# TXH-mercury/VALOR

Hardware: AMD Instinct MI355X
Metric: pretrain samples/sec (V+A+T clip) (higher is better)
Workload: dtype bf16

## Files before the change

include/valor_hip.h:

```cpp
#ifndef VALOR_HIP_H
#define VALOR_HIP_H
#include <stdint.h>
#ifdef __cplusplus
extern "C" {
#endif

#define VALOR_DT_BF16 0
#define VALOR_DT_F32 1
#define VALOR_OK 0
#define VALOR_ERR_ARG (-1)
#define VALOR_ERR_LAUNCH (-2)
#define VALOR_ACT_NONE 0
#define VALOR_ACT_GELU_ERF 1
#define VALOR_ACT_QUICK_GELU 2
#define VALOR_ACT_RELU 3
#define VALOR_ACT_TANH 4
#define VALOR_ACT_DERIV 16

int valor_gemm(void* stream, int dtype, int transA, int transB, int M, int N, int K, const void* A, int64_t lda,
               const void* B, int64_t ldb, void* C, int64_t ldc, const void* bias, int act, void* preact,
               const void* dact_aux, int64_t ldaux, float alpha, int accumulate, int out_f32, void* workspace,
               int64_t workspace_bytes, void* rowsum_out,
               int rowsum_accumulate);

typedef struct valor_gemm_policy {
    int key[12];
    int variant;
    int tr_asm;
    int fast_epilogue;
    int sched_256;
    int sched_narrow;
} valor_gemm_policy;
int valor_gemm_tuned(const valor_gemm_policy* policy, void* stream, int dtype, int transA, int transB, int M, int N, int K,
                     const void* A, int64_t lda, const void* B, int64_t ldb, void* C, int64_t ldc, const void* bias, int act,
                     void* preact, const void* dact_aux, int64_t ldaux, float alpha, int accumulate, int out_f32, void* workspace,
                     int64_t workspace_bytes, void* rowsum_out, int rowsum_accumulate);
int valor_gemm_kernel_for_tuned(const valor_gemm_policy* policy, int dtype, int transA, int transB, int M, int N, int K,
                                int heavy_epilogue);

typedef struct valor_gemm_pending { unsigned char opaque[256]; } valor_gemm_pending;
int valor_gemm_deferred(void* stream, int dtype, int transA, int transB, int M, int N, int K, const void* A, int64_t lda,
                        const void* B, int64_t ldb, void* C, int64_t ldc, const void* bias, int act, void* preact,
                        const void* dact_aux, int64_t ldaux, float alpha, int accumulate, int out_f32, void* workspace,
                        int64_t workspace_bytes, void* rowsum_out, int rowsum_accumulate, valor_gemm_pending* pending);
int valor_gemm_pending_bytes(const valor_gemm_pending* pending, int64_t* bytes);
int valor_gemm_reduce_group(void* stream, int dtype, const valor_gemm_pending* pendings, int n);

int valor_gemm_set_variant(int v);
int valor_gemm_kernel_for(int dtype, int transA, int transB, int M, int N, int K, int heavy_epilogue);
int valor_gemm_set_tr_asm(int v);
int valor_gemm_set_fast_epilogue(int v);
int valor_gemm_set_policy(int key, int value);
int valor_gemm_set_8ph_sched(int v);
int valor_gemm_set_narrow_sched(int v);
int valor_gemm_narrow_occupancy(void);
int valor_gemm_wide_occupancy(void);

typedef struct valor_xattn_seg {
    const void* q; const void* o; const void* dout; void* dq; const float* lse; const int* kv_range;
    int64_t q_bs, q_rs, o_bs, o_rs, do_bs, do_rs, dq_bs, dq_rs;
    int B, Sq;
    uint64_t seed, offset;
} valor_xattn_seg;
int valor_cross_attn_fwd_fused(void* stream, int dtype, const valor_xattn_seg* segs, int nseg, const void* k, const void* v, int H, int Skv,
                               int kv_bmod, int64_t k_bs, int64_t k_rs, int64_t v_bs, int64_t v_rs, float scale, float p_drop,
                               const uint64_t* rng_base);
int valor_cross_attn_bwd_fused(void* stream, int dtype, const valor_xattn_seg* segs, int nseg, const void* k, const void* v, void* dk, void* dv,
                               int H, int Skv, int kv_bmod, int64_t k_bs, int64_t k_rs, int64_t v_bs, int64_t v_rs, int64_t dk_bs,
                               int64_t dk_rs, int64_t dv_bs, int64_t dv_rs, float scale, float p_drop, const uint64_t* rng_base);

int valor_ln_part_blocks(void);
int valor_ln_set_variant(int v);
int valor_ln_set_nt(int v);
int valor_bdrln_fwd(void* stream, int dtype, const void* x, const void* bias, const void* residual, const void* gamma,
                    const void* beta, void* z, void* y, float* mean, float* rstd, int64_t rows, int cols, float eps,
                    float p_drop, uint64_t seed, uint64_t offset, const float* row_scale, int64_t rows_per_scale,
                    const uint64_t* rng_base);
int valor_bdrln_bwd(void* stream, int dtype, const void* dy, const void* dz_in, const void* z, const float* mean,
                    const float* rstd, const void* gamma, void* dx, void* dres, float* part_dgamma, float* part_dbeta,
                    float* part_dbias, int64_t rows, int cols, float p_drop, uint64_t seed, uint64_t offset, const float* row_scale,
                    int64_t rows_per_scale, const uint64_t* rng_base);
int valor_colsum_finalize(void* stream, int dtype, const float* part, int nparts, int cols, void* out, int out_f32,
                          int accumulate);
int valor_colsum_finalize3(void* stream, int dtype, const float* part0, void* out0, int acc0, const float* part1, void* out1,
                           int acc1, const float* part2, void* out2, int acc2, int nparts, int cols);
int valor_colsum(void* stream, int dtype, const void* x, int64_t rows, int cols, int64_t ld, float* part, void* out,
                 int out_f32, int accumulate);

int valor_attn_set_variant(int v);
int valor_attn_decode_fwd(void* stream, int dtype, const void* q, const void* k, const void* v, void* o, float* lse,
                          int B, int H, int Sq, int Skv, int64_t q_bs, int64_t q_rs, int64_t k_bs, int64_t k_rs,
                          int64_t v_bs, int64_t v_rs, int64_t o_bs, int64_t o_rs, const float* mask, int64_t mask_bs,
                          int64_t mask_rs, const int* key_row, int64_t key_row_bs, float scale);
int valor_attn_set_res_pipeline(int v);

int valor_attn_fwd(void* stream, int dtype, const void* q, const void* k, const void* v, void* o, float* lse, int B,
                   int H, int Sq, int Skv, int64_t q_bs, int64_t q_rs, int64_t k_bs, int64_t k_rs, int64_t v_bs,
                   int64_t v_rs, int64_t o_bs, int64_t o_rs, const float* mask, int64_t mask_bs, int64_t mask_rs,
                   const int* kv_range, int kv_bmod, float scale, float p_drop, uint64_t seed, uint64_t offset,
                   const uint64_t* rng_base);
int valor_attn_bwd(void* stream, int dtype, const void* q, const void* k, const void* v, const void* o, const float* lse,
                   const void* dout, void* dq, void* dk, void* dv, float* delta, int B, int H, int Sq, int Skv,
                   int64_t q_bs, int64_t q_rs, int64_t k_bs, int64_t k_rs, int64_t v_bs, int64_t v_rs, int64_t o_bs,
                   int64_t o_rs, int64_t do_bs, int64_t do_rs, int64_t dq_bs, int64_t dq_rs, int64_t dk_bs, int64_t dk_rs,
                   int64_t dv_bs, int64_t dv_rs, const float* mask, int64_t mask_bs, int64_t mask_rs, const int* kv_range,
// ... 193 lines not shown
```

valor_amd/build.py:

```python
import hashlib
import os
import subprocess
import sys
from concurrent.futures import ThreadPoolExecutor

HERE = os.path.dirname(os.path.abspath(__file__))
CSRC = os.path.join(HERE, "csrc")
LIB = os.path.join(HERE, "libvalor_hip.so")
OBJDIR = os.path.join(CSRC, "_obj")
PUBLIC_HEADER = os.path.join(os.path.dirname(HERE), "include", "valor_hip.h")
HIPCC = os.environ.get("HIPCC", "/opt/rocm/bin/hipcc")
FLAGS = ["--offload-arch=gfx950", "-O3", "-std=c++17", "-fPIC", "-Wno-unused-value", "-Wno-unused-result"]


HOT_KERNELS = ("gemm_8ph_kernel", "gemm_8ph2_kernel", "gemm_glds_kernel", "gemm_splitk_reduce", "attn_res_", "attn_x_", "attn_xu_", "ln_fwd", "ln_bwd", "adamw_kernel", "xent_",
               "fine_fused_fwd", "fine_fused_fwd_fp8_kernel", "fine_ds_chunk_kernelIDF16bLi16", "win_fwd", "win_bwd_dkv", "topk_segment_kernel",
               "topk_merge_kernel", "fine_score_pairs_kernel", "grad_partial_kernel", "update_partial_kernel", "ema_kernel", "trie_constrain_kernel",
               "trie_score_level_kernel")
KNOWN_SCRATCH = ("attn_x_fwd_kernelILi8", "attn_x_bwd_kernelILi4ELb1",
                 "kernelIf")


def _sources():
    return sorted(f for f in os.listdir(CSRC) if f.endswith(".hip"))


def _headers_digest():
    h = hashlib.sha1()
    for f in sorted(os.listdir(CSRC)):
        if f.endswith(".h"):
            with open(os.path.join(CSRC, f), "rb") as fh:
                h.update(fh.read())
    with open(PUBLIC_HEADER, "rb") as fh:
        h.update(fh.read())
    return h.hexdigest()


def _compile_one(src, hdig, verbose):
    path = os.path.join(CSRC, src)
    obj = os.path.join(OBJDIR, src[:-4] + ".o")
    stamp = obj + ".sha1"
    with open(path, "rb") as fh:
        dig = hashlib.sha1(fh.read() + hdig.encode() + " ".join(FLAGS).encode()).hexdigest()
    if os.path.exists(obj) and os.path.exists(stamp) and open(stamp).read() == dig:
        return obj, False
    cmd = [HIPCC] + FLAGS + ["-Rpass-analysis=kernel-resource-usage", "-c", path, "-o", obj]
    if verbose:
        print("[valor_amd.build]", " ".join(cmd), flush=True)
    r = subprocess.run(cmd, capture_output=True, text=True)
    if r.returncode != 0:
        sys.stderr.write(r.stdout + r.stderr)
        raise RuntimeError(f"hipcc failed on {src}")
    fn = None
    bad = []
    for line in r.stderr.splitlines():
        if "Function Name:" in line:
            fn = line.split("Function Name:")[1].split()[0]
        elif "ScratchSize [bytes/lane]:" in line:
            n = int(line.split("ScratchSize [bytes/lane]:")[1].split()[0])
            if n:
                hot = any(h in fn for h in HOT_KERNELS) and not any(k in fn for k in KNOWN_SCRATCH)
                print(f"[valor_amd.build] {'ERROR' if hot else 'WARNING'}: {src}: kernel {fn} uses {n} B/lane of scratch", flush=True)
                if hot:
                    bad.append(fn)
    if bad and os.environ.get("VALOR_BUILD_STRICT", "1") != "0":
        raise RuntimeError(f"scratch in hot kernels of {src}: {bad} (see -Rpass-analysis=kernel-resource-usage; VALOR_BUILD_STRICT=0 builds anyway)")
    with open(stamp, "w") as fh:
        fh.write(dig)
# ... 28 lines not shown
```

valor_amd/csrc/gemm.hip:

```cpp
#include "gemm_common.h"
#include <stdlib.h>

template <typename T, bool TA, bool TB>
__global__ __launch_bounds__(256) void gemm_kernel(GemmArgs p) {
    constexpr int VEC = ElemTraits<T>::VEC;
    constexpr int BK = 8 * VEC;
    constexpr int TILE_BYTES = 128 * TILE_ROW_BYTES;
    extern __shared__ __attribute__((aligned(16))) char smem[];

    const int tid = threadIdx.x;
    const int lane = tid & 63;
    const int wave = __builtin_amdgcn_readfirstlane(tid >> 6);
    const int wm = wave >> 1, wn = wave & 1;

    const int tiles_n = (p.N + 127) >> 7;
    const int tiles_m = (p.M + 127) >> 7;
    const int logical = xcd_remap(blockIdx.x, tiles_m * tiles_n);
    const int tm = logical / tiles_n, tn = logical - tm * tiles_n;
    const int m0 = tm << 7, n0 = tn << 7;

    const int nk_total = (p.K + BK - 1) / BK;
    int ks_begin = 0, ks_end = nk_total;
    if (p.kslices > 1) {
        ks_begin = blockIdx.y * p.ksteps_per_slice;
// ... 360 lines not shown
        const int n = (int)(i - (int64_t)m * nquads) << 2;
        f32x4_t s = {0.f, 0.f, 0.f, 0.f};
        if (p.ws_bf16) {
            for (int k = 0; k < p.kslices; ++k) {
                const bf16_t* q = (const bf16_t*)p.ws + ((int64_t)k * p.M + m) * p.N + n;
                if (n + 3 < p.N && (p.N & 3) == 0) s += load4<bf16_t>(q);
                else for (int r = 0; r < 4; ++r) if (n + r < p.N) s[r] += (float)q[r];
            }
        } else {
            for (int k = 0; k < p.kslices; ++k) {
                const float* q = p.ws + ((int64_t)k * p.M + m) * p.N + n;
                if (n + 3 < p.N && (p.N & 3) == 0) s += *(const f32x4_t*)q;
                else for (int r = 0; r < 4; ++r) if (n + r < p.N) s[r] += q[r];
            }
        }
        epilogue_store<T>(p, m, n, s, load_bias4<T>(p, n));
    }
    }
    if (p.rowsum_out) {
        for (int m = bid * blockDim.x + threadIdx.x; m < p.M; m += nblk * blockDim.x) {
            float t = 0.f;
            for (int k = 0; k < p.kslices; ++k) t += p.rowsum_ws[(int64_t)k * p.M + m];
            rowsum_store<T>(p, m, t);
        }
    }
}
template <typename T>
__global__ __launch_bounds__(256) void gemm_splitk_reduce(GemmArgs p) {
    splitk_reduce_body<T>(p, blockIdx.x, gridDim.x);
}

#define VALOR_REDUCE_GROUP 8
struct ReduceGroupArgs {
    GemmArgs g[VALOR_REDUCE_GROUP];
    int first[VALOR_REDUCE_GROUP + 1];
    int n;
};
template <typename T>
__global__ __launch_bounds__(256) void gemm_splitk_reduce_group(ReduceGroupArgs a) {
    int i = 0;
    while (i + 1 < a.n && (int)blockIdx.x >= a.first[i + 1]) ++i;
    splitk_reduce_body<T>(a.g[i], blockIdx.x - a.first[i], a.first[i + 1] - a.first[i]);
}
static int reduce_blocks(const GemmArgs& p) {
    const int64_t total = (int64_t)p.M * ((p.N + 3) / 4);
    int blocks = (int)((total + 255) / 256);
    return blocks > 4096 ? 4096 : blocks;
}

static int g_gemm_variant = 4;
static inline int gemm_variant() { return GEMM_KNOB(variant, g_gemm_variant); }
extern "C" int valor_gemm_set_variant(int v) { const int o = g_gemm_variant; if (v >= 0 && v <= 4) g_gemm_variant = v; return o; }
thread_local const GemmTuning* t_gemm_tuning = nullptr;
int g_gemm_policy_default[12] = {[] { const char* e = getenv("VALOR_GEMM_NT_MINK"); return e ? atoi(e) : 768; }(),
                        [] { const char* e = getenv("VALOR_GEMM_SPLITK_BF16"); return e ? atoi(e) : 1; }(),
                        [] { const char* e = getenv("VALOR_GEMM_MIN_TILES"); return e ? atoi(e) : 256; }(),
                        [] { const char* e = getenv("VALOR_GEMM_NT_MIN_TILES"); return e ? atoi(e) : 1024; }(),
                        [] { const char* e = getenv("VALOR_GEMM_RASTER"); return e ? atoi(e) : 1000; }(),
                        [] { const char* e = getenv("VALOR_GEMM_STORE"); return e ? atoi(e) : 1000; }(),
                        [] { const char* e = getenv("VALOR_GEMM_NTA"); return e ? atoi(e) : 0; }(),
                        [] { const char* e = getenv("VALOR_GEMM_NN_MINK"); return e ? atoi(e) : 128; }(),
                        [] { const char* e = getenv("VALOR_GEMM_NARROW"); return e ? atoi(e) : 1000; }(),
                        [] { const char* e = getenv("VALOR_GEMM_MFMA32"); return e ? atoi(e) : 0; }(),
                        [] { const char* e = getenv("VALOR_GEMM_WIDE"); return e ? atoi(e) : 0; }(),
                        [] { const char* e = getenv("VALOR_GEMM_SKINNY_ALL"); return e ? atoi(e) : 0; }()};
extern "C" int valor_gemm_set_policy(int key, int value) {
    if (key < 0 || key > 11) return VALOR_ERR_ARG;
    const int old = g_gemm_policy_default[key];
    if (value >= 0) g_gemm_policy_default[key] = value;
    return old;
}

static bool use_8ph(int dtype, int transA, int transB, int M, int N, int K, bool heavy_epi = false) {
    if (dtype != VALOR_DT_BF16 || gemm_variant() < 3) return false;
    if ((K % 64) != 0 || K < 128 || M < 256 || N < 256) return false;
    if (gemm_variant() == 3) return true;
    const int64_t tiles256 = (int64_t)((M + 255) / 256) * ((N + 255) / 256);
    if (transA && transB) return K >= 4096;
    if (!transA && !transB) return tiles256 >= gemm_policy(2) && K >= gemm_policy(7);
    if (!transA && transB) return tiles256 >= gemm_policy(3) && K >= (heavy_epi ? 1536 : gemm_policy(0));
    return false;
}

static bool use_8ph2(int dtype, int transA, int transB, int M, int N, int K, bool heavy_epi, bool big) {
    const int mode = gemm_policy(8);
    if (dtype != VALOR_DT_BF16 || gemm_variant() != 4 || mode == 0) return false;
    if ((K % 64) != 0 || K < 128 || M < 256 || N < 128) return false;
    if (transA && !transB) return false;
    if (mode == 1) return true;
    if (mode == 2) return !big;
    if (mode == 3) return big;
    (void)heavy_epi;
    if (transA) return false;
    if (!big) return true;
    const int64_t tiles256 = (int64_t)((M + 255) / 256) * ((N + 255) / 256);
    return K <= 1024 && (N >= 1536 || tiles256 < 1024);
}

static int gemm_family(int dtype, int transA, int transB, int M, int N, int K, bool heavy_epi) {
    if (dtype != VALOR_DT_BF16 || gemm_variant() == 0) return 0;
    if (gemm_variant() == 4 && !transA && !transB && M <= gemm_policy(11) && N >= 16 && gemm_skinny_chunks(K)) return 5;
    const bool big = use_8ph(dtype, transA, transB, M, N, K, heavy_epi);
    if (use_8ph2(dtype, transA, transB, M, N, K, heavy_epi, big)) return 4;
    if (big) return 3;
    return gemm_variant() == 2 ? 2 : 1;
}

extern "C" int valor_gemm_kernel_for(int dtype, int transA, int transB, int M, int N, int K, int heavy_epilogue) {
    return gemm_family(dtype, transA, transB, M, N, K, heavy_epilogue != 0);
}
struct TuningScope {
    const GemmTuning* prev;
    explicit TuningScope(const void* t) : prev(t_gemm_tuning) { if (t) t_gemm_tuning = (const GemmTuning*)t; }
    ~TuningScope() { t_gemm_tuning = prev; }
};
static_assert(sizeof(GemmTuning) == 17 * sizeof(int), "valor_gemm_policy layout (include/valor_hip.h)");
extern "C" int valor_gemm_kernel_for_tuned(const void* policy, int dtype, int transA, int transB, int M, int N, int K, int heavy_epilogue) {
    TuningScope scope(policy);
    return gemm_family(dtype, transA, transB, M, N, K, heavy_epilogue != 0);
}

template <int NSTAGE>
static void launch_gemm_glds(hipStream_t st, int transA, int transB, const GemmArgs& p, dim3 grid) {
    const size_t lds = NSTAGE * 32768;
#define VALOR_GLDS_LAUNCH1(TA_, TB_, F_, W_)                                                        \
    do {                                                                                            \
        static bool attr_set = false;                                                               \
        if (!attr_set) {                                                                            \
            hipFuncSetAttribute((const void*)gemm_glds_kernel<TA_, TB_, NSTAGE, F_, W_>,            \
                                hipFuncAttributeMaxDynamicSharedMemorySize, (int)lds);              \
            attr_set = true;                                                                        \
        }                                                                                           \
        hipLaunchKernelGGL((gemm_glds_kernel<TA_, TB_, NSTAGE, F_, W_>), grid, dim3(256), lds, st, p); \
    } while (0)
#define VALOR_GLDS_LAUNCH(TA_, TB_)                                                                 \
    do {                                                                                            \
        if constexpr (NSTAGE == 1) {                                                                \
            if (fused) VALOR_GLDS_LAUNCH1(TA_, TB_, true, 3);                                       \
            else VALOR_GLDS_LAUNCH1(TA_, TB_, false, 4);                                            \
        } else {                                                                                    \
            if (fused) VALOR_GLDS_LAUNCH1(TA_, TB_, true, 2);                                       \
            else VALOR_GLDS_LAUNCH1(TA_, TB_, false, 2);                                            \
        }                                                                                           \
    } while (0)
    const bool fused = p.kslices <= 1 && ((p.act & VALOR_ACT_MASK) != VALOR_ACT_NONE || p.preact || p.dact_aux);
    if (!transA && !transB) VALOR_GLDS_LAUNCH(false, false);
    else if (!transA && transB) VALOR_GLDS_LAUNCH(false, true);
    else if (transA && !transB) VALOR_GLDS_LAUNCH(true, false);
    else VALOR_GLDS_LAUNCH(true, true);
#undef VALOR_GLDS_LAUNCH
#undef VALOR_GLDS_LAUNCH1
}

template <typename T>
static int launch_gemm(hipStream_t st, int transA, int transB, GemmArgs p) {
    const int tiles = ((p.M + 127) / 128) * ((p.N + 127) / 128);
    dim3 grid(tiles, p.kslices > 1 ? p.kslices : 1);
    if (ElemTraits<T>::DT == VALOR_DT_BF16 && gemm_variant() > 0) {
        if (p.kslices > 1) grid = dim3(tiles * p.kslices, 1);
        const int fam = gemm_family(VALOR_DT_BF16, transA, transB, p.M, p.N, p.K, p.dact_aux != nullptr && !(p.act & VALOR_ACT_DERIV));
        if (fam == 4) launch_gemm_8ph2(st, transA, transB, p);
        else if (fam == 3) launch_gemm_8ph(st, transA, transB, p);
        else {
            p.st_mode = (gemm_policy(6) && !p.out_f32 && p.kslices <= 1 && p.K <= 1024 && (int64_t)p.M * p.N >= (4 << 20)) ? 1 : 0;
            if (gemm_variant() == 2) launch_gemm_glds<2>(st, transA, transB, p, grid);
            else launch_gemm_glds<1>(st, transA, transB, p, grid);
        }
        if (p.kslices > 1 && !p.defer_reduce)
            hipLaunchKernelGGL((gemm_splitk_reduce<T>), dim3(reduce_blocks(p)), dim3(256), 0, st, p);
        return valor_launch_status();
    }
    const size_t lds = 2 * 2 * 128 * TILE_ROW_BYTES;
#define VALOR_GEMM_LAUNCH(TA_, TB_)                                                               \
    do {                                                                                          \
        static bool attr_set = false;                                                             \
        if (!attr_set) {                                                                          \
            hipFuncSetAttribute((const void*)gemm_kernel<T, TA_, TB_>,                            \
                                hipFuncAttributeMaxDynamicSharedMemorySize, (int)lds);            \
            attr_set = true;                                                                      \
        }                                                                                         \
        hipLaunchKernelGGL((gemm_kernel<T, TA_, TB_>), grid, dim3(256), lds, st, p);              \
    } while (0)
    if (!transA && !transB) VALOR_GEMM_LAUNCH(false, false);
    else if (!transA && transB) VALOR_GEMM_LAUNCH(false, true);
    else if (transA && !transB) VALOR_GEMM_LAUNCH(true, false);
    else VALOR_GEMM_LAUNCH(true, true);
#undef VALOR_GEMM_LAUNCH
    if (p.kslices > 1 && !p.defer_reduce)
        hipLaunchKernelGGL((gemm_splitk_reduce<T>), dim3(reduce_blocks(p)), dim3(256), 0, st, p);
    return valor_launch_status();
}

struct PendingBlob { GemmArgs p; int dtype; int valid; };
static_assert(sizeof(PendingBlob) <= 256, "valor_gemm_pending is 256 bytes");

static int gemm_impl(void* stream, int dtype, int transA, int transB, int M, int N, int K,
                     const void* A, int64_t lda, const void* B, int64_t ldb, void* C, int64_t ldc,
                     const void* bias, int act, void* preact, const void* dact_aux, int64_t ldaux,
                     float alpha, int accumulate, int out_f32, void* workspace, int64_t workspace_bytes,
                     void* rowsum_out, int rowsum_accumulate, PendingBlob* pending);

extern "C" int valor_gemm(void* stream, int dtype, int transA, int transB, int M, int N, int K,
                          const void* A, int64_t lda, const void* B, int64_t ldb, void* C, int64_t ldc,
                          const void* bias, int act, void* preact, const void* dact_aux, int64_t ldaux,
                          float alpha, int accumulate, int out_f32, void* workspace, int64_t workspace_bytes,
                          void* rowsum_out, int rowsum_accumulate) {
    return gemm_impl(stream, dtype, transA, transB, M, N, K, A, lda, B, ldb, C, ldc, bias, act, preact, dact_aux, ldaux, alpha, accumulate,
                     out_f32, workspace, workspace_bytes, rowsum_out, rowsum_accumulate, nullptr);
}

extern "C" int valor_gemm_tuned(const void* policy, void* stream, int dtype, int transA, int transB, int M, int N, int K,
                                const void* A, int64_t lda, const void* B, int64_t ldb, void* C, int64_t ldc,
                                const void* bias, int act, void* preact, const void* dact_aux, int64_t ldaux,
                                float alpha, int accumulate, int out_f32, void* workspace, int64_t workspace_bytes,
                                void* rowsum_out, int rowsum_accumulate) {
    TuningScope scope(policy);
// ... 159 lines not shown
```

valor_amd/csrc/gemm_common.h:

```cpp
#pragma once
#include "mma.h"

struct GemmArgs {
    const void* A; const void* B; void* C;
    const void* bias;
    void* preact;
    const void* dact_aux;
    float* ws;
    int64_t lda, ldb, ldc, ldaux;
    int M, N, K;
    int act;
    int accumulate;
    int out_f32;
    int kslices;
    int ksteps_per_slice;
    float alpha;
    uint32_t bytesA, bytesB;
    void* rowsum_out;
    float* rowsum_ws;
    int rowsum_acc;
    int fast_epi;
    int raster_g;
    int st_mode;
    int ws_bf16;
// ... 131 lines not shown
    if (!vec8) {
        epilogue_store<T, FUSED>(p, m, n0, a0, b0);
        epilogue_store<T, FUSED>(p, m, n0 + 4, a1, b1);
        return;
    }
    const int64_t off = (int64_t)m * p.ldc + n0;
    f32x4_t v0, v1;
#pragma unroll
    for (int r = 0; r < 4; ++r) { v0[r] = a0[r] * p.alpha + b0[r]; v1[r] = a1[r] * p.alpha + b1[r]; }
    if constexpr (FUSED) {
        const int act = p.act & VALOR_ACT_MASK;
        const bool deriv = (p.act & VALOR_ACT_DERIV) != 0;
        f32x4_t q0 = v0, q1 = v1;
        if ((act != VALOR_ACT_NONE || (deriv && p.preact)) && !p.dact_aux) {
            float f[8] = {v0[0], v0[1], v0[2], v0[3], v1[0], v1[1], v1[2], v1[3]};
            if (p.preact && deriv) {
                float g[8];
                act_fwd_deriv_n<8>(act, f, g);
                q0 = (f32x4_t){g[0], g[1], g[2], g[3]};
                q1 = (f32x4_t){g[4], g[5], g[6], g[7]};
            } else {
                act_fwd_n<8>(act, f);
            }
            v0 = (f32x4_t){f[0], f[1], f[2], f[3]};
            v1 = (f32x4_t){f[4], f[5], f[6], f[7]};
        }
        if (p.preact) {
            u32x4_t q = {pack2_bf16(q0[0], q0[1]), pack2_bf16(q0[2], q0[3]), pack2_bf16(q1[0], q1[1]), pack2_bf16(q1[2], q1[3])};
            if constexpr (NTS < 0) store_out16(p.st_mode, (T*)p.preact + off, q);
            else store_out16<NTS != 0>((T*)p.preact + off, q);
        }
        if (p.dact_aux) {
            const T* a = (const T*)p.dact_aux + (int64_t)m * p.ldaux + n0;
            const f32x4_t u0 = load4<T>(a), u1 = load4<T>(a + 4);
            if (deriv) {
                v0 *= u0; v1 *= u1;
            } else {
                float f[8] = {v0[0], v0[1], v0[2], v0[3], v1[0], v1[1], v1[2], v1[3]};
                const float x[8] = {u0[0], u0[1], u0[2], u0[3], u1[0], u1[1], u1[2], u1[3]};
                act_bwd_mul_n<8>(act, f, x);
                v0 = (f32x4_t){f[0], f[1], f[2], f[3]};
                v1 = (f32x4_t){f[4], f[5], f[6], f[7]};
            }
        }
    }
    T* c = (T*)p.C + off;
    if (p.accumulate) { v0 += load4<T>(c); v1 += load4<T>(c + 4); }
    u32x4_t o = {pack2_bf16(v0[0], v0[1]), pack2_bf16(v0[2], v0[3]), pack2_bf16(v1[0], v1[1]), pack2_bf16(v1[2], v1[3])};
    if constexpr (NTS < 0) store_out16(p.st_mode, c, o);
    else store_out16<NTS != 0>(c, o);
}

void launch_gemm_8ph(hipStream_t st, int transA, int transB, const GemmArgs& p);
void launch_gemm_8ph2(hipStream_t st, int transA, int transB, const GemmArgs& p);
void launch_gemm_8w(hipStream_t st, const GemmArgs& p, int tiles, bool nts);
int gemm_skinny_chunks(int K);
int launch_gemm_skinny(hipStream_t st, const GemmArgs& p);
struct GemmTuning { int key[12]; int variant, tr_asm, fast_epilogue, sched_256, sched_narrow; };
extern thread_local const GemmTuning* t_gemm_tuning;
extern int g_gemm_policy_default[12];
static inline int gemm_policy(int k) {
    const GemmTuning* o = t_gemm_tuning;
    return (o && o->key[k] >= 0) ? o->key[k] : g_gemm_policy_default[k];
}
#define GEMM_KNOB(FIELD_, GLOBAL_) ((t_gemm_tuning && t_gemm_tuning->FIELD_ >= 0) ? t_gemm_tuning->FIELD_ : (GLOBAL_))
int gemm_tr_asm_now();
int gemm_fast_epilogue_now();
```

valor_amd/lib.py:

```python
import ctypes
import os

_HERE = os.path.dirname(os.path.abspath(__file__))
LIB_PATH = os.environ.get("VALOR_HIP_LIB") or os.path.join(_HERE, "libvalor_hip.so")

DT_BF16 = 0
DT_F32 = 1

ACT_NONE, ACT_GELU_ERF, ACT_QUICK_GELU, ACT_RELU, ACT_TANH = 0, 1, 2, 3, 4
ACT_DERIV = 16

_c = ctypes
_vp, _i, _i64, _u64, _f = _c.c_void_p, _c.c_int, _c.c_int64, _c.c_uint64, _c.c_float

class GemmPolicy(_c.Structure):
    _fields_ = [("key", _i * 12), ("variant", _i), ("tr_asm", _i), ("fast_epilogue", _i), ("sched_256", _i), ("sched_narrow", _i)]
    KEYS = dict(nt_min_k=0, splitk_bf16=1, min_tiles=2, nt_min_tiles=3, raster=4, store=5, nta=6, nn_min_k=7, narrow=8, mfma32=9, wide=10, skinny=11)

    @classmethod
    def make(cls, **kw):
        p = cls()
        for i in range(12):
            p.key[i] = -1
        p.variant = p.tr_asm = p.fast_epilogue = p.sched_256 = p.sched_narrow = -1
        for k, v in kw.items():
            if k in cls.KEYS:
                p.key[cls.KEYS[k]] = int(v)
            else:
                setattr(p, k, int(v))
        return p


class XattnSeg(_c.Structure):
    _fields_ = [("q", _vp), ("o", _vp), ("dout", _vp), ("dq", _vp), ("lse", _vp), ("kv_range", _vp),
                ("q_bs", _i64), ("q_rs", _i64), ("o_bs", _i64), ("o_rs", _i64), ("do_bs", _i64), ("do_rs", _i64), ("dq_bs", _i64), ("dq_rs", _i64),
                ("B", _i), ("Sq", _i), ("seed", _u64), ("offset", _u64)]


class RewardTables(_c.Structure):
    POINTERS = ("g_keys", "g_idf", "clip_ref_ptr", "ref_key_ptr", "ref_keys", "ref_vals", "ref_norm", "ref_bigrams", "ref_tokens",
                "clip_bleu_ptr", "bleu_keys", "bleu_cnt")
    _fields_ = [(k, _vp) for k in POINTERS] + [("ref_len", _c.c_double), ("n_global", _c.c_int32), ("n_clips", _c.c_int32)]


class CapevalTables(_c.Structure):
    POINTERS = RewardTables.POINTERS + ("ref_sym_ptr", "ref_syms")
    _fields_ = [(k, _vp) for k in POINTERS] + [("ref_len", _c.c_double), ("n_global", _c.c_int32), ("n_clips", _c.c_int32)]


class CapevalSummary(_c.Structure):
    _fields_ = [("value", _c.c_double * 6), ("total", _c.c_int64 * 10)]


SIGNATURES = {
    "valor_gemm": [_vp, _i, _i, _i, _i, _i, _i, _vp, _i64, _vp, _i64, _vp, _i64, _vp, _i, _vp, _vp, _i64,
                   _f, _i, _i, _vp, _i64, _vp, _i],
    "valor_gemm_tuned": [_vp, _vp, _i, _i, _i, _i, _i, _i, _vp, _i64, _vp, _i64, _vp, _i64, _vp, _i, _vp, _vp, _i64,
                         _f, _i, _i, _vp, _i64, _vp, _i],
    "valor_gemm_kernel_for_tuned": [_vp, _i, _i, _i, _i, _i, _i, _i],
    "valor_gemm_deferred": [_vp, _i, _i, _i, _i, _i, _i, _vp, _i64, _vp, _i64, _vp, _i64, _vp, _i, _vp, _vp, _i64,
                            _f, _i, _i, _vp, _i64, _vp, _i, _vp],
    "valor_gemm_pending_bytes": [_vp, _vp],
    "valor_gemm_reduce_group": [_vp, _i, _vp, _i],
    "valor_gemm_set_variant": [_i],
    "valor_gemm_kernel_for": [_i, _i, _i, _i, _i, _i, _i],
    "valor_gemm_set_tr_asm": [_i],
    "valor_gemm_set_fast_epilogue": [_i],
    "valor_gemm_set_policy": [_i, _i],
    "valor_gemm_set_8ph_sched": [_i],
    "valor_gemm_set_narrow_sched": [_i],
    "valor_gemm_narrow_occupancy": [],
    "valor_gemm_wide_occupancy": [],
    "valor_ln_part_blocks": [],
    "valor_ln_set_variant": [_i],
    "valor_ln_set_nt": [_i],
    "valor_bdrln_fwd": [_vp, _i, _vp, _vp, _vp, _vp, _vp, _vp, _vp, _vp, _vp, _i64, _i, _f, _f, _u64, _u64, _vp, _i64, _vp],
    "valor_bdrln_bwd": [_vp, _i, _vp, _vp, _vp, _vp, _vp, _vp, _vp, _vp, _vp, _vp, _vp, _i64, _i, _f, _u64, _u64, _vp, _i64, _vp],
    "valor_patchify3d": [_vp, _i, _vp, _vp, _i, _i, _i, _i, _i, _i],
    "valor_group_mean_fwd": [_vp, _i, _vp, _vp, _i64, _i, _i],
    "valor_group_mean_bwd": [_vp, _i, _vp, _vp, _i64, _i, _i],
    "valor_win_attn_workspace_floats": [_i, _i, _i, _i],
    "valor_win_attn_set_variant": [_i],
    "valor_win_attn_fwd": [_vp, _i, _vp, _vp, _vp, _vp, _vp, _vp, _vp, _i, _i, _i, _i, _i, _i, _i, _f],
    "valor_win_attn_bwd": [_vp, _i, _vp, _vp, _vp, _vp, _vp, _vp, _vp, _vp, _vp, _vp, _vp, _vp, _i, _vp, _i64, _i, _i, _i, _i, _i, _i, _i, _f],
    "valor_colsum_finalize": [_vp, _i, _vp, _i, _i, _vp, _i, _i],
    "valor_colsum_finalize3": [_vp, _i, _vp, _vp, _i, _vp, _vp, _i, _vp, _vp, _i, _i, _i],
    "valor_attn_set_variant": [_i],
    "valor_attn_set_res_pipeline": [_i],
    "valor_attn_fwd": [_vp, _i, _vp, _vp, _vp, _vp, _vp, _i, _i, _i, _i, _i64, _i64, _i64, _i64, _i64, _i64, _i64, _i64,
                       _vp, _i64, _i64, _vp, _i, _f, _f, _u64, _u64, _vp],
    "valor_attn_decode_fwd": [_vp, _i, _vp, _vp, _vp, _vp, _vp, _i, _i, _i, _i, _i64, _i64, _i64, _i64, _i64, _i64, _i64, _i64,
                              _vp, _i64, _i64, _vp, _i64, _f],
    "valor_attn_bwd": [_vp, _i, _vp, _vp, _vp, _vp, _vp, _vp, _vp, _vp, _vp, _vp, _i, _i, _i, _i,
                       _i64, _i64, _i64, _i64, _i64, _i64, _i64, _i64, _i64, _i64, _i64, _i64, _i64, _i64, _i64, _i64,
                       _vp, _i64, _i64, _vp, _i, _f, _f, _u64, _u64, _i, _vp],
    "valor_cross_attn_fwd_fused": [_vp, _i, _vp, _i, _vp, _vp, _i, _i, _i, _i64, _i64, _i64, _i64, _f, _f, _vp],
    "valor_cross_attn_bwd_fused": [_vp, _i, _vp, _i, _vp, _vp, _vp, _vp, _i, _i, _i, _i64, _i64, _i64, _i64, _i64, _i64, _i64, _i64, _f, _f, _vp],
    "valor_reducer_unique_id": [_vp],
    "valor_reducer_create": [_vp, _vp, _i, _i, _i, _vp, _vp, _vp, _i, _i],
    "valor_reducer_launch_bucket": [_vp, _i, _vp, _i],
    "valor_reducer_wait": [_vp, _vp],
    "valor_reducer_destroy": [_vp],
    "valor_xent_fwd": [_vp, _i, _vp, _vp, _vp, _vp, _i64, _i, _i64],
    "valor_xent_bwd": [_vp, _i, _vp, _vp, _vp, _vp, _f, _i64, _i, _i64],
    "valor_xent_smooth_fwd": [_vp, _i, _vp, _vp, _vp, _vp, _i64, _i, _i64, _f],
    "valor_xent_smooth_bwd": [_vp, _i, _vp, _vp, _vp, _vp, _f, _i64, _i, _i64, _f],
    "valor_fine_weight_softmax": [_vp, _vp, _vp, _vp, _i, _i],
    "valor_fine_weight_softmax_bwd": [_vp, _vp, _vp, _vp, _i, _i],
    "valor_fine_reduce_fwd": [_vp, _vp, _i64, _vp, _vp, _vp, _vp, _vp, _vp, _vp, _vp, _vp, _i, _i, _i],
    "valor_fine_scores": [_vp, _vp, _i64, _vp, _vp, _vp, _vp, _vp, _i, _i, _i, _i],
    "valor_infonce_fwd": [_vp, _vp, _vp, _vp, _vp, _vp, _i],
    "valor_infonce_bwd": [_vp, _vp, _vp, _vp, _vp, _vp, _vp, _vp, _vp, _i],
    "valor_fine_reduce_bwd": [_vp, _i, _vp, _vp, _vp, _vp, _vp, _vp, _vp, _vp, _vp, _vp, _i64, _vp, _vp, _i, _i, _i],
    "valor_fine_fused_fwd": [_vp, _vp, _vp, _vp, _vp, _vp, _vp, _vp, _vp, _vp, _vp, _vp, _i, _i, _i, _i, _i],
    "valor_fine_ds_chunk": [_vp, _i, _vp, _vp, _vp, _vp, _vp, _vp, _vp, _vp, _i64, _i, _i, _i, _i, _i],
    "valor_fine_weight_grad": [_vp, _vp, _vp, _vp, _vp, _vp, _i, _i, _i],
    "valor_fine_set_fused": [_i],
    "valor_retrieval_workspace_bytes": [_i, _i, _c.POINTER(_i64)],
# ... 87 lines not shown
```

Measured before the change: 558.1.

## Add quadrant-scheduled 256x256 GEMM kernel for long-K TN×TN family-3 shapes

Adds a new bf16 GEMM kernel (gemm_8q) that splits each 256x256 tile into four 128x128 quadrants and interleaves LDS fragment reads and global-to-LDS DMA for the next k-tile inside the MFMA stream, with a barrier per quadrant phase. It is used for family-3 GEMMs with both operands transposed when the per-workgroup k-tile count exceeds 48, and this is on by default through a new policy key. The aim is to hide memory latency better on long-K GEMMs than the existing 8ph kernel does. In exchange it adds more barriers and higher register pressure from the 8x8 accumulator plus four fragment sets, and it is a second kernel path to maintain.

Result: faster. 564.7, median of 6 (+1.2%).

```diff
diff --git a/include/valor_hip.h b/include/valor_hip.h
--- a/include/valor_hip.h
+++ b/include/valor_hip.h
@@ -51,6 +51,7 @@
 int valor_gemm_set_tr_asm(int v);
 int valor_gemm_set_fast_epilogue(int v);
 int valor_gemm_set_policy(int key, int value);
+int valor_gemm_wave128_for(int dtype, int transA, int transB, int M, int N, int K, int heavy_epilogue);
 int valor_gemm_set_8ph_sched(int v);
 int valor_gemm_set_narrow_sched(int v);
 int valor_gemm_narrow_occupancy(void);
diff --git a/valor_amd/build.py b/valor_amd/build.py
--- a/valor_amd/build.py
+++ b/valor_amd/build.py
@@ -13,7 +13,7 @@
 FLAGS = ["--offload-arch=gfx950", "-O3", "-std=c++17", "-fPIC", "-Wno-unused-value", "-Wno-unused-result"]
 
 
-HOT_KERNELS = ("gemm_8ph_kernel", "gemm_8ph2_kernel", "gemm_glds_kernel", "gemm_splitk_reduce", "attn_res_", "attn_x_", "attn_xu_", "ln_fwd", "ln_bwd", "adamw_kernel", "xent_",
+HOT_KERNELS = ("gemm_8ph_kernel", "gemm_8q_kernel", "gemm_8ph2_kernel", "gemm_glds_kernel", "gemm_splitk_reduce", "attn_res_", "attn_x_", "attn_xu_", "ln_fwd", "ln_bwd", "adamw_kernel", "xent_",
                "fine_fused_fwd", "fine_fused_fwd_fp8_kernel", "fine_ds_chunk_kernelIDF16bLi16", "win_fwd", "win_bwd_dkv", "topk_segment_kernel",
                "topk_merge_kernel", "fine_score_pairs_kernel", "grad_partial_kernel", "update_partial_kernel", "ema_kernel", "trie_constrain_kernel",
                "trie_score_level_kernel")
diff --git a/valor_amd/csrc/gemm.hip b/valor_amd/csrc/gemm.hip
--- a/valor_amd/csrc/gemm.hip
+++ b/valor_amd/csrc/gemm.hip
@@ -436,7 +436,7 @@
 static inline int gemm_variant() { return GEMM_KNOB(variant, g_gemm_variant); }
 extern "C" int valor_gemm_set_variant(int v) { const int o = g_gemm_variant; if (v >= 0 && v <= 4) g_gemm_variant = v; return o; }
 thread_local const GemmTuning* t_gemm_tuning = nullptr;
-int g_gemm_policy_default[12] = {[] { const char* e = getenv("VALOR_GEMM_NT_MINK"); return e ? atoi(e) : 768; }(),
+int g_gemm_policy_default[13] = {[] { const char* e = getenv("VALOR_GEMM_NT_MINK"); return e ? atoi(e) : 768; }(),
                         [] { const char* e = getenv("VALOR_GEMM_SPLITK_BF16"); return e ? atoi(e) : 1; }(),
                         [] { const char* e = getenv("VALOR_GEMM_MIN_TILES"); return e ? atoi(e) : 256; }(),
                         [] { const char* e = getenv("VALOR_GEMM_NT_MIN_TILES"); return e ? atoi(e) : 1024; }(),
@@ -447,9 +447,10 @@
                         [] { const char* e = getenv("VALOR_GEMM_NARROW"); return e ? atoi(e) : 1000; }(),
                         [] { const char* e = getenv("VALOR_GEMM_MFMA32"); return e ? atoi(e) : 0; }(),
                         [] { const char* e = getenv("VALOR_GEMM_WIDE"); return e ? atoi(e) : 0; }(),
-                        [] { const char* e = getenv("VALOR_GEMM_SKINNY_ALL"); return e ? atoi(e) : 0; }()};
+                        [] { const char* e = getenv("VALOR_GEMM_SKINNY_ALL"); return e ? atoi(e) : 0; }(),
+                        [] { const char* e = getenv("VALOR_GEMM_WAVE128"); return e ? atoi(e) : 1000; }()};
 extern "C" int valor_gemm_set_policy(int key, int value) {
-    if (key < 0 || key > 11) return VALOR_ERR_ARG;
+    if (key < 0 || key > 12) return VALOR_ERR_ARG;
     const int old = g_gemm_policy_default[key];
     if (value >= 0) g_gemm_policy_default[key] = value;
     return old;
@@ -488,6 +489,28 @@
     if (use_8ph2(dtype, transA, transB, M, N, K, heavy_epi, big)) return 4;
     if (big) return 3;
     return gemm_variant() == 2 ? 2 : 1;
+}
+
+static int family3_ktiles_per_workgroup(int M, int N, int K) {
+    const int nk = K / 64, tiles = ((M + 255) / 256) * ((N + 255) / 256);
+    int sl = 1;
+    if (2 * tiles <= 256 && nk >= 24) {
+        sl = 256 / tiles;
+        if (sl > nk / 6) sl = nk / 6;
+        if (sl > 64) sl = 64;
+        if (sl < 2) sl = 1;
+    }
+    return (nk + sl - 1) / sl;
+}
+static bool use_wave128(int dtype, int transA, int transB, int M, int N, int K, bool heavy_epi) {
+    const int mode = gemm_policy(12);
+    if (mode == 0 || gemm_family(dtype, transA, transB, M, N, K, heavy_epi) != 3) return false;
+    if (!(transA && transB)) return false;
+    if (mode == 1) return true;
+    return family3_ktiles_per_workgroup(M, N, K) > 48;
+}
+extern "C" int valor_gemm_wave128_for(int dtype, int transA, int transB, int M, int N, int K, int heavy_epilogue) {
+    return use_wave128(dtype, transA, transB, M, N, K, heavy_epilogue != 0) ? 1 : 0;
 }
 
 extern "C" int valor_gemm_kernel_for(int dtype, int transA, int transB, int M, int N, int K, int heavy_epilogue) {
@@ -544,8 +567,10 @@
         if (p.kslices > 1) grid = dim3(tiles * p.kslices, 1);
         const int fam = gemm_family(VALOR_DT_BF16, transA, transB, p.M, p.N, p.K, p.dact_aux != nullptr && !(p.act & VALOR_ACT_DERIV));
         if (fam == 4) launch_gemm_8ph2(st, transA, transB, p);
-        else if (fam == 3) launch_gemm_8ph(st, transA, transB, p);
-        else {
+        else if (fam == 3) {
+            if (use_wave128(VALOR_DT_BF16, transA, transB, p.M, p.N, p.K, p.dact_aux != nullptr && !(p.act & VALOR_ACT_DERIV))) launch_gemm_8q(st, transA, transB, p);
+            else launch_gemm_8ph(st, transA, transB, p);
+        } else {
             p.st_mode = (gemm_policy(6) && !p.out_f32 && p.kslices <= 1 && p.K <= 1024 && (int64_t)p.M * p.N >= (4 << 20)) ? 1 : 0;
             if (gemm_variant() == 2) launch_gemm_glds<2>(st, transA, transB, p, grid);
             else launch_gemm_glds<1>(st, transA, transB, p, grid);
diff --git a/valor_amd/csrc/gemm8q.hip b/valor_amd/csrc/gemm8q.hip
--- /dev/null
+++ b/valor_amd/csrc/gemm8q.hip
@@ -0,0 +1,310 @@
+#include "gemm_common.h"
+#include <stdlib.h>
+
+#define HT_BYTES 16384
+#define BUF_BYTES (4 * HT_BYTES)
+#define OFF_A0 0
+#define OFF_A1 HT_BYTES
+#define OFF_B0 (2 * HT_BYTES)
+#define OFF_B1 (3 * HT_BYTES)
+
+template <bool KSLOW> struct FragSet;
+template <> struct FragSet<false> { bf16x8_t f[4][2]; };
+template <> struct FragSet<true> { TrPair f[4][2]; };
+DEVINL bf16x8_t frag_of(const bf16x8_t& f) { return f; }
+DEVINL bf16x8_t frag_of(const TrPair& t) { return tr_frag(t); }
+DEVINL void mfma_acc(f32x4_t& c, bf16x8_t a, bf16x8_t b) { asm("v_mfma_f32_16x16x32_bf16 %0, %1, %2, %0" : "+a"(c) : "v"(a), "v"(b)); }
+DEVINL void mfma_rowsum(f32x4_t& r0, f32x4_t& r1, bf16x8_t ones, bf16x8_t f0, bf16x8_t f1, bf16x8_t f2, bf16x8_t f3, int sel) {
+    asm volatile("s_cmp_lt_i32 %7, 1\n\ts_cbranch_scc1 2f\n\ts_cmp_eq_u32 %7, 1\n\ts_cbranch_scc0 1f\n\t"
+                 "v_mfma_f32_16x16x32_bf16 %0, %2, %3, %0\n\tv_mfma_f32_16x16x32_bf16 %1, %2, %4, %1\n\ts_branch 2f\n"
+                 "1:\n\tv_mfma_f32_16x16x32_bf16 %0, %2, %5, %0\n\tv_mfma_f32_16x16x32_bf16 %1, %2, %6, %1\n"
+                 "2:"
+                 : "+v"(r0), "+v"(r1) : "v"(ones), "v"(f0), "v"(f1), "v"(f2), "v"(f3), "s"(sel) : "scc");
+}
+DEVINL void wait8(FragSet<false>&) { asm volatile("s_waitcnt lgkmcnt(0)" ::: "memory"); }
+DEVINL void wait8(FragSet<true>& s) { tr_wait8(s.f); }
+DEVINL void wait4(FragSet<false>&, int) { asm volatile("s_waitcnt lgkmcnt(0)" ::: "memory"); }
+DEVINL void wait4(FragSet<true>& s, int kk) { tr_wait_4(s.f[0][kk], s.f[1][kk], s.f[2][kk], s.f[3][kk]); }
+
+template <bool TA, bool TB>
+__global__ __launch_bounds__(256) void gemm_8q_kernel(GemmArgs p) {
+    typedef bf16_t T;
+    constexpr int BK = 64;
+    extern __shared__ __attribute__((aligned(16))) char smem[];
+
+    const int tid = threadIdx.x;
+    const int lane = tid & 63;
+    const int wave = __builtin_amdgcn_readfirstlane(tid >> 6);
+    const int wm = wave >> 1, wn = wave & 1;
+    const int fr = lane & 15, fg = lane >> 4;
+
+    const int tiles_n = (p.N + 255) >> 8;
+    const int tiles_m = (p.M + 255) >> 8;
+    int logical, slice = 0;
+    if (p.kslices > 1) {
+        const int ntiles = tiles_m * tiles_n;
+        const int item = xcd_remap(blockIdx.x, ntiles * p.kslices);
+        slice = item / ntiles;
+        logical = item - slice * ntiles;
+    } else {
+        logical = xcd_remap(blockIdx.x, tiles_m * tiles_n);
+    }
+    int tm = logical / tiles_n, tn = logical - tm * tiles_n;
+    if (p.raster_g > 0 && p.kslices <= 1) {
+        const int G = p.raster_g, per = G * tiles_m;
+        const int grp = logical / per, w = logical - grp * per;
+        const int gw = min(G, tiles_n - grp * G);
+        tm = w / gw;
+        tn = grp * G + (w - tm * gw);
+    }
+    const int m0 = tm << 8, n0 = tn << 8;
+
+    const int nk_total = p.K / BK;
+    int ks_begin = 0, ks_end = nk_total;
+    if (p.kslices > 1) {
+        ks_begin = slice * p.ksteps_per_slice;
+        ks_end = ks_begin + p.ksteps_per_slice;
+        if (ks_end > nk_total) ks_end = nk_total;
+        if (ks_begin > nk_total) ks_begin = nk_total;
+    }
+    const int k_first = ks_begin * BK;
+    const int ntile = ks_end - ks_begin;
+
+    f32x4_t acc[8][8];
+#pragma unroll
+    for (int i = 0; i < 8; ++i)
+#pragma unroll
+        for (int j = 0; j < 8; ++j) acc[i][j] = (f32x4_t){0.f, 0.f, 0.f, 0.f};
+
+    const bool do_rs = TA && p.rowsum_out != nullptr && tn == 0;
+    f32x4_t racc[2][2];
+#pragma unroll
+    for (int i = 0; i < 2; ++i)
+#pragma unroll
+        for (int j = 0; j < 2; ++j) racc[i][j] = (f32x4_t){0.f, 0.f, 0.f, 0.f};
+    bf16x8_t ones = __builtin_bit_cast(bf16x8_t, (u32x4_t){0x3f803f80u, 0x3f803f80u, 0x3f803f80u, 0x3f803f80u});
+    asm volatile("" : "+v"(ones));
+    const int rs_sel = __builtin_amdgcn_readfirstlane(do_rs ? wn + 1 : 0);
+
+    int oA[2][4], oB[2][4];
+    int stepA, stepB;
+    {
+        const int ldA_b = (int)(p.lda * 2), ldB_b = (int)(p.ldb * 2);
+#pragma unroll
+        for (int hf = 0; hf < 2; ++hf)
+#pragma unroll
+            for (int i = 0; i < 4; ++i) {
+                const int pc = wave * 4 + i;
+                if constexpr (!TA) {
+                    const int r = pc * 8 + (lane >> 3), c = (lane & 7) ^ ((lane >> 3) & 7);
+                    oA[hf][i] = (m0 + hf * 128 + r) * ldA_b + (k_first + c * 8) * 2;
+                } else {
+                    const int k = pc * 4 + (lane >> 4), s = lane & 15;
+                    const int ic = ((s - 2 * (k & 3) - 8 * ((k >> 3) & 1)) & 15) * 8;
+                    oA[hf][i] = (k_first + k) * ldA_b + (m0 + hf * 128 + ic) * 2;
+                }
+                if constexpr (!TB) {
+                    const int r = pc * 8 + (lane >> 3), c = (lane & 7) ^ ((lane >> 3) & 7);
+                    oB[hf][i] = (n0 + hf * 128 + r) * ldB_b + (k_first + c * 8) * 2;
+                } else {
+                    const int k = pc * 4 + (lane >> 4), s = lane & 15;
+                    const int ic = ((s - 2 * (k & 3) - 8 * ((k >> 3) & 1)) & 15) * 8;
+                    oB[hf][i] = (k_first + k) * ldB_b + (n0 + hf * 128 + ic) * 2;
+                }
+            }
+        stepA = TA ? BK * ldA_b : BK * 2;
+        stepB = TB ? BK * ldB_b : BK * 2;
+    }
+    auto dmaA = [&](int hf, char* buf, int t, int i) {
+        const rsrc_t rs = make_rsrc(p.A, t < ntile ? p.bytesA : 0u);
+        glds16(rs, buf + (hf ? OFF_A1 : OFF_A0) + wave * 4096 + i * 1024, oA[hf][i]);
+        oA[hf][i] += stepA; asm volatile("" : "+v"(oA[hf][i]));
+    };
+    auto dmaB = [&](int hf, char* buf, int t, int i) {
+        const rsrc_t rs = make_rsrc(p.B, t < ntile ? p.bytesB : 0u);
+        glds16(rs, buf + (hf ? OFF_B1 : OFF_B0) + wave * 4096 + i * 1024, oB[hf][i]);
+        oB[hf][i] += stepB; asm volatile("" : "+v"(oB[hf][i]));
+    };
+
+    int trA[4], trB[4];
+    {
+        const int base = (8 * fg + (fr >> 2)) * 256 + 8 * (fr & 1);
+        const int rot = 2 * (fr >> 2) + 8 * (fg & 1);
+#pragma unroll
+        for (int i = 0; i < 4; ++i) {
+            trA[i] = base + 16 * ((2 * (wm * 4 + i) + ((fr >> 1) & 1) + rot) & 15);
+            trB[i] = base + 16 * ((2 * (wn * 4 + i) + ((fr >> 1) & 1) + rot) & 15);
+        }
+    }
+    auto rdA = [&](const char* img, FragSet<TA>& s, int mt, int kk) {
+        if constexpr (TA) tr_issue(s.f[mt][kk], img + trA[mt] + kk * (32 * 256));
+        else s.f[mt][kk] = read_frag<T>(img, wm * 64 + mt * 16 + fr, kk * 4 + fg);
+    };
+    auto rdB = [&](const char* img, FragSet<TB>& s, int nt, int kk) {
+        if constexpr (TB) tr_issue(s.f[nt][kk], img + trB[nt] + kk * (32 * 256));
+        else s.f[nt][kk] = read_frag<T>(img, wn * 64 + nt * 16 + fr, kk * 4 + fg);
+    };
+#define PIN() __builtin_amdgcn_sched_barrier(0)
+    auto quadrant = [&](int mh, int nh, FragSet<TA>& sa, FragSet<TB>& sb, auto&& slot) __attribute__((always_inline)) {
+#pragma unroll
+        for (int kk = 0; kk < 2; ++kk)
+#pragma unroll
+            for (int mt = 0; mt < 4; ++mt)
+#pragma unroll
+                for (int nt = 0; nt < 4; ++nt) {
+                    const int i = kk * 16 + mt * 4 + nt;
+                    mfma_acc(acc[mh * 4 + mt][nh * 4 + nt], frag_of(sb.f[nt][kk]), frag_of(sa.f[mt][kk]));
+                    slot(i);
+                    PIN();
+                }
+    };
+    auto rowsum = [&](int hh, FragSet<TA>& sa) __attribute__((always_inline)) {
+        if constexpr (TA) {
+#pragma unroll
+            for (int kk = 0; kk < 2; ++kk)
+                mfma_rowsum(racc[hh][0], racc[hh][1], ones, frag_of(sa.f[0][kk]), frag_of(sa.f[1][kk]), frag_of(sa.f[2][kk]), frag_of(sa.f[3][kk]), rs_sel);
+            PIN();
+        }
+    };
+#define PHASE_END()                                                                                               \
+    do {                                                                                                          \
+        asm volatile("s_waitcnt vmcnt(20)" ::: "memory");                                                         \
+        __builtin_amdgcn_s_barrier();                                                                             \
+        PIN();                                                                                                    \
+    } while (0)
+
+    FragSet<TA> fax, fay;
+    FragSet<TB> fb0, fb1;
+    if (ntile > 0) {
+#pragma unroll
+        for (int t = 0; t < 2; ++t) {
+            char* const b = smem + t * BUF_BYTES;
+#pragma unroll
+            for (int i = 0; i < 4; ++i) dmaA(0, b, t, i);
+#pragma unroll
+            for (int i = 0; i < 4; ++i) dmaB(0, b, t, i);
+#pragma unroll
+            for (int i = 0; i < 4; ++i) dmaB(1, b, t, i);
+#pragma unroll
+            for (int i = 0; i < 4; ++i) dmaA(1, b, t, i);
+        }
+        PIN();
+        PHASE_END();
+#pragma unroll
+        for (int i = 0; i < 8; ++i) rdA(smem + OFF_A0, fax, i & 3, i >> 2);
+#pragma unroll
+        for (int i = 0; i < 4; ++i) rdB(smem + OFF_B0, fb0, i, 0);
+        PIN();
+        wait8(fax); wait4(fb0, 0);
+        __builtin_amdgcn_s_barrier();
+        PIN();
+        for (int rel = 0; rel < ntile; ++rel) {
+            char* const cur = smem + (rel & 1) * BUF_BYTES;
+            char* const nxt = smem + ((rel & 1) ^ 1) * BUF_BYTES;
+            quadrant(0, 0, fax, fb0, [&](int i) {
+                if (i < 4) rdB(cur + OFF_B0, fb0, i, 1);
+                else if (i < 8) dmaA(0, cur, rel + 2, i - 4);
+                else if (i == 15) { PIN(); wait4(fb0, 1); }
+                else if (i >= 16 && i < 24) rdB(cur + OFF_B1, fb1, i & 3, (i - 16) >> 2);
+            });
+            rowsum(0, fax);
+            PIN();
+            wait8(fb1);
+            PHASE_END();
+            quadrant(0, 1, fax, fb1, [&](int i) {
+                if (i < 8) rdA(cur + OFF_A1, fay, i & 3, i >> 2);
+                else if (i < 16 && !(i & 1)) dmaB(0, cur, rel + 2, (i - 8) >> 1);
+            });
+            PIN();
+            wait8(fay);
+            PHASE_END();
+            quadrant(1, 1, fay, fb1, [&](int i) {
+                if (i < 4) rdA(nxt + OFF_A0, fax, i, 0);
+                else if (i >= 8 && i < 16 && !(i & 1)) dmaB(1, cur, rel + 2, (i - 8) >> 1);
+            });
+            rowsum(1, fay);
+            PIN();
+            wait4(fax, 0);
+            PHASE_END();
+            quadrant(1, 0, fay, fb0, [&](int i) {
+                if (i < 4) rdA(nxt + OFF_A0, fax, i, 1);
+                else if (i >= 8 && i < 16 && !(i & 1)) dmaA(1, cur, rel + 2, (i - 8) >> 1);
+                else if (i >= 16 && i < 20) rdB(nxt + OFF_B0, fb0, i - 16, 0);
+            });
+            PIN();
+            wait4(fax, 1); wait4(fb0, 0);
+            PHASE_END();
+        }
+    }
+    asm volatile("s_nop 15\n\ts_nop 15\n\ts_waitcnt vmcnt(0)" ::: "memory");
+    PIN();
+    __syncthreads();
+#undef PHASE_END
+#undef PIN
+    if (do_rs && fg == 0) {
+#pragma unroll
+        for (int hh = 0; hh < 2; ++hh)
+#pragma unroll
+            for (int i = 0; i < 2; ++i) {
+                const int m = m0 + hh * 128 + wm * 64 + (2 * wn + i) * 16 + fr;
+                if (m < p.M) {
+                    if (p.kslices > 1) p.rowsum_ws[(int64_t)slice * p.M + m] = racc[hh][i][0];
+                    else rowsum_store<T>(p, m, racc[hh][i][0]);
+                }
+            }
+    }
+
+    float* sC = (float*)smem;
+    float* wsl = p.kslices > 1 ? p.ws + (int64_t)slice * p.M * p.N : nullptr;
+    const f32x4_t bias0 = load_bias4<T>(p, n0 + (tid & 31) * 8), bias1 = load_bias4<T>(p, n0 + (tid & 31) * 8 + 4);
+#pragma unroll
+    for (int pass = 0; pass < 2; ++pass) {
+        if (pass) __syncthreads();
+#pragma unroll
+        for (int mt = 0; mt < 4; ++mt)
+#pragma unroll
+            for (int ni = 0; ni < 8; ++ni) {
+                const int ml = wm * 64 + mt * 16 + fr;
+                const int ch = ((ni >> 2) * 32 + wn * 16 + (ni & 3) * 4 + fg) ^ (ml & 7);
+                *(f32x4_t*)(sC + ml * 256 + ch * 4) = acc[pass * 4 + mt][ni];
+            }
+        __syncthreads();
+#pragma unroll 2
+        for (int it = 0; it < 16; ++it) {
+            const int ml = it * 8 + (tid >> 5);
+            const int c8 = tid & 31;
+            const f32x4_t v0 = *(const f32x4_t*)(sC + ml * 256 + (((2 * c8) ^ (ml & 7)) << 2));
+            const f32x4_t v1 = *(const f32x4_t*)(sC + ml * 256 + (((2 * c8 + 1) ^ (ml & 7)) << 2));
+            const int m = m0 + pass * 128 + ml, n = n0 + c8 * 8;
+            if (wsl) {
+                splitk_store8(p, slice, m, n, v0, v1);
+            } else {
+                epilogue_store8<true, 0>(p, m, n, v0, v1, bias0, bias1);
+            }
+        }
+    }
+}
+
+void launch_gemm_8q(hipStream_t st, int transA, int transB, const GemmArgs& p_in) {
+    GemmArgs p = p_in;
+    p.fast_epi = 0;
+    p.raster_g = 0;
+    p.st_mode = 0;
+    const int tiles = ((p.M + 255) / 256) * ((p.N + 255) / 256);
+    dim3 grid(tiles * (p.kslices > 1 ? p.kslices : 1));
+    const size_t lds = 2 * BUF_BYTES;
+#define VALOR_8Q_LAUNCH(TA_, TB_)                                                                               \
+    do {                                                                                                        \
+        static bool attr_set = false;                                                                           \
+        if (!attr_set) {                                                                                        \
+            hipFuncSetAttribute((const void*)gemm_8q_kernel<TA_, TB_>, hipFuncAttributeMaxDynamicSharedMemorySize, (int)lds); \
+            attr_set = true;                                                                                    \
+        }                                                                                                       \
+        hipLaunchKernelGGL((gemm_8q_kernel<TA_, TB_>), grid, dim3(256), lds, st, p);                            \
+    } while (0)
+    if (transA && transB) VALOR_8Q_LAUNCH(true, true);
+    else if (!transA && !transB) VALOR_8Q_LAUNCH(false, false);
+    else if (!transA && transB) VALOR_8Q_LAUNCH(false, true);
+    else VALOR_8Q_LAUNCH(true, false);
+#undef VALOR_8Q_LAUNCH
+}
diff --git a/valor_amd/csrc/gemm_common.h b/valor_amd/csrc/gemm_common.h
--- a/valor_amd/csrc/gemm_common.h
+++ b/valor_amd/csrc/gemm_common.h
@@ -207,16 +207,17 @@
 }
 
 void launch_gemm_8ph(hipStream_t st, int transA, int transB, const GemmArgs& p);
+void launch_gemm_8q(hipStream_t st, int transA, int transB, const GemmArgs& p);
 void launch_gemm_8ph2(hipStream_t st, int transA, int transB, const GemmArgs& p);
 void launch_gemm_8w(hipStream_t st, const GemmArgs& p, int tiles, bool nts);
 int gemm_skinny_chunks(int K);
 int launch_gemm_skinny(hipStream_t st, const GemmArgs& p);
 struct GemmTuning { int key[12]; int variant, tr_asm, fast_epilogue, sched_256, sched_narrow; };
 extern thread_local const GemmTuning* t_gemm_tuning;
-extern int g_gemm_policy_default[12];
+extern int g_gemm_policy_default[13];
 static inline int gemm_policy(int k) {
     const GemmTuning* o = t_gemm_tuning;
-    return (o && o->key[k] >= 0) ? o->key[k] : g_gemm_policy_default[k];
+    return (o && k < 12 && o->key[k] >= 0) ? o->key[k] : g_gemm_policy_default[k];
 }
 #define GEMM_KNOB(FIELD_, GLOBAL_) ((t_gemm_tuning && t_gemm_tuning->FIELD_ >= 0) ? t_gemm_tuning->FIELD_ : (GLOBAL_))
 int gemm_tr_asm_now();
diff --git a/valor_amd/lib.py b/valor_amd/lib.py
--- a/valor_amd/lib.py
+++ b/valor_amd/lib.py
@@ -64,6 +64,7 @@
     "valor_gemm_reduce_group": [_vp, _i, _vp, _i],
     "valor_gemm_set_variant": [_i],
     "valor_gemm_kernel_for": [_i, _i, _i, _i, _i, _i, _i],
+    "valor_gemm_wave128_for": [_i, _i, _i, _i, _i, _i, _i],
     "valor_gemm_set_tr_asm": [_i],
     "valor_gemm_set_fast_epilogue": [_i],
     "valor_gemm_set_policy": [_i, _i],
```
